# GRatTWCU/Social-STGCNN

Hardware: AMD Instinct MI355X
Metric: scene-windows/sec fwd+bwd (obs=8,pred=12) (higher is better)
Workload: dtype f32; 1 GPU; synthetic V=32 scene-windows, obs 8 / pred 12, batch 2048 per GPU, f32 (BASELINE north-star: V<=32, batch=2048; SURVEY 8d generator); global_batch=2048, step=aggregation + forward + bivariate NLL + backward + SGD update, parallelism=dp1

## Files before the change

### social_stgcnn_amd/csrc/model_bwd.hip

```cpp
#include "model_common.hpp"
#include "stgcn_block.hpp"
#include "txp_scene_common.hpp"
#include "step_plan.hpp"
#include "txp_wgrad.hpp"
#include "tail_parts.hpp"
#include "nll_elem.hpp"

namespace stg {

struct BwdArgs {
    ModelLayout lay;
    const float *params, *buffers, *x;
    int64_t x_sn, x_sc, x_st, x_sv;
    const float *adj;
    int64_t a_sn;
    const int32_t *num_peds;
    int N, V;
    const float *dy, *ws;
    const float *nll_target, *nll_weights;
    float *nll_losses;
    int64_t ws_stride;
    float *slab1;
    float *dzg;
    float *dx;
// ... 221 lines not shown
                const int r = e / vi, w = e - r * vi;
                dcur[e] = dyn[(int64_t)r * V + w];
            }
            __syncthreads();
        }
        float *H1 = dzb, *DH2 = dzb + C * (T + 2) * Vl, *DB1 = DH2 + C * (T + 2) * Vl;
        for (int j = L.n_blocks - 1; j >= 0 && !STG_SKIP(a, 4); --j) {
            const float *xin = j > 0 ? wsn + L.ws_hdr_floats + (int64_t)L.blk[j - 1].ws_s * V : nullptr;
            float *dxs = j > 0 ? dcur : nullptr;
            float *dxg = j == 0 ? dxn : nullptr;
            if (L.blk[j].cin == Cfg::CIN0)
                stgcn_block_bwd<Cfg::CIN0, WAVES, true>(a, params, L.blk[j], n, vi, dcur, H1, DH2, DB1, red, tot, gsm, wsn,
                                                        xin, dxs, dxg, nullptr);
            else
                stgcn_block_bwd<Cfg::C, WAVES, true>(a, params, L.blk[j], n, vi, dcur, H1, DH2, DB1, red, tot, gsm, wsn, xin,
                                                     dxs, dxg, nullptr);
        }
    }
    __syncthreads();
    float *slab = a.slab1 + (int64_t)blockIdx.x * n_small;
    for (int e = tid; e < n_small; e += NT) slab[e] = gsm[e];
}

struct ReduceSeg {
    int p0, len, rows, row_stride;
    int64_t base;
};
struct ReduceArgs {
    ReduceSeg seg[kMaxTxp + 3];
    int n_seg;
    const float *slabs;
    float *grad;
    int n_params;
};

struct TailArgs {
    float *params;
    const float *lr_dev;
    float lr;
    const float *stats, *losses, *weights;
    const int32_t *num_peds;
    float *buffers, *total;
    NbtPtrs nbt;
    int n_reduce, n_buffers, N, stat_floats;
    float momentum;
};

__global__ __launch_bounds__(256) void reduce_slabs_kernel(const ReduceArgs a, const TailArgs t_) {
    __shared__ float part[32][8];
    if ((int)blockIdx.x >= t_.n_reduce) {
        float *acc_s = &part[0][0];
        __shared__ float dec_s[256];
        __shared__ int cnt_s[256];
        const int b = (int)blockIdx.x - t_.n_reduce;
        if (b < t_.n_buffers)
            bn_fold_body<256>(b, t_.stats, t_.num_peds, t_.N, t_.stat_floats, t_.momentum, t_.buffers, t_.nbt, acc_s, dec_s,
                              cnt_s);
        else if (t_.total)
            weighted_sum_body(t_.losses, t_.weights, t_.N, t_.total, acc_s);
        return;
    }
    const int col = threadIdx.x & 7, grp = threadIdx.x >> 3;
    const int p = blockIdx.x * 8 + col;
    float s = 0.f;
    if (p < a.n_params) {
        for (int q = 0; q < a.n_seg; ++q) {
            const ReduceSeg g = a.seg[q];
            if (p >= g.p0 && p < g.p0 + g.len) {
                const float *src = a.slabs + g.base + (p - g.p0);
                int k = grp;
                for (; k + 992 < g.rows; k += 1024) {
                    float v[32];
#pragma unroll
                    for (int u = 0; u < 32; ++u) v[u] = src[(int64_t)(k + 32 * u) * g.row_stride];
#pragma unroll
                    for (int u = 0; u < 32; ++u) s += v[u];
                }
                for (; k + 480 < g.rows; k += 512) {
                    float v[16];
#pragma unroll
                    for (int u = 0; u < 16; ++u) v[u] = src[(int64_t)(k + 32 * u) * g.row_stride];
#pragma unroll
                    for (int u = 0; u < 16; ++u) s += v[u];
                }
                for (; k + 96 < g.rows; k += 128) {
                    float v[4];
#pragma unroll
                    for (int u = 0; u < 4; ++u) v[u] = src[(int64_t)(k + 32 * u) * g.row_stride];
#pragma unroll
                    for (int u = 0; u < 4; ++u) s += v[u];
                }
                for (; k < g.rows; k += 32) s += src[(int64_t)k * g.row_stride];
            }
        }
    }
    part[grp][col] = s;
    __syncthreads();
    if (grp == 0 && p < a.n_params) {
        float t = 0.f;
#pragma unroll
        for (int g = 0; g < 32; ++g) t += part[g][col];
        a.grad[p] = t;
        if (t_.params) t_.params[p] -= (t_.lr_dev ? t_.lr_dev[0] : t_.lr) * t;
    }
}

static int env_waves(const char *name, int dflt) {
    const int w = diag_env(name, dflt);
    return (w == 1 || w == 2 || w == 4 || w == 8) ? w : dflt;
}

static size_t bwd_lds_bytes(const ModelLayout &L, int V, int waves) {
    const int plane = Cfg::P * txp_sc(V);
    const int st = (2 * Cfg::C * (Cfg::T + 2) + Cfg::C * Cfg::T) * V;
    const int reg = plane > st ? plane : st;
    const int dcur = Cfg::P * Cfg::C * V;
    const int n_small = L.n_blk_params + L.n_txp;
    const size_t fl = ((n_small + 3) & ~3) + (size_t)reg + (size_t)dcur + (size_t)waves * kRedMax + kRedMax;
    return fl * sizeof(float);
}

static int bwd_waves(const StepPath &path, int V) {
    return path.wg_waves ? path.wg_waves : (V <= 40 ? 1 : (V <= 80 ? 4 : 8));
}

static int bwd_grid_w(const ModelLayout &L, int N, int V, int waves) {
    const size_t lds = bwd_lds_bytes(L, V, waves);
// ... 91 lines not shown
        return STG_EUNSUPPORTED;
    STG_REQUIRE(!(path.scene() && dx), STG_EUNSUPPORTED,
                "stg_model_bwd: dx is only computed by the workgroup-per-scene kernels: set STG_OPT_WG_PATH in the "
                "descriptor of the forward and the backward call");
    a.params = params; a.buffers = buffers; a.x = x;
    a.x_sn = x_sn; a.x_sc = x_sc; a.x_st = x_st; a.x_sv = x_sv;
    a.adj = adj; a.a_sn = a_sn; a.num_peds = num_peds; a.N = N; a.V = V;
    a.nll_target = nll_target; a.nll_weights = nll_weights; a.nll_losses = nll_losses;
    a.dy = dy; a.ws = ws; a.ws_stride = ws_floats_per_scene(L, V); a.slab1 = rows; a.dzg = dzg; a.dx = dx;
    int32_t *order = reinterpret_cast<int32_t *>(scratch + cv.order);
    bool sorted;
    const WsTail wt = ws_tail(L, path, N, V);
    const float *ws_end = ws + wt.base;
    if (tail_has_order(path, num_peds, N, V)) {
        order = reinterpret_cast<int32_t *>(const_cast<float *>(ws_end) + wt.order);
        sorted = true;
    } else {
        sorted = launch_scene_order(num_peds, N, V, order, order + N, st, order + N + V + 2);
    }
    int32_t *order_peds = order + N + V + 2;
    const int serp = diag_env("STG_WALK", 1);
    a.tier = SceneTier{sorted ? order : nullptr, sorted ? order + N : nullptr, -1, V, serp};
    a.debug_skip = diag_env("STG_DEBUG_SKIP", 0);
    int slab_rows;
    if (path.scene()) {
        TxpBwdArgs t{};
        t.lay = L; t.params = params; t.num_peds = num_peds; t.N = N; t.V = V; t.dy = dy; t.ws = ws;
        t.nll_target = nll_target; t.nll_weights = nll_weights; t.nll_losses = nll_losses;
        t.x = x; t.x_sn = x_sn; t.x_sc = x_sc; t.x_st = x_st; t.x_sv = x_sv; t.adj = adj; t.a_sn = a_sn;
        t.ws_stride = a.ws_stride; t.dzg = dzg; t.rows = rows;
        t.tier = a.tier;
        t.Vl = V;
        t.debug_skip = a.debug_skip;
        t.split_bf16 = (L.flags & STG_OPT_SPLIT_BF16) ? 1 : 0;
        t.stagger = diag_env("STG_STAGGER_B", 0);
        if (wt.wp >= 0) t.wp = reinterpret_cast<const unsigned *>(ws_end + wt.wp);
        const int rcw = launch_scene_bwd(path, t, st);
        if (rcw != STG_OK) return rcw;
        slab_rows = N;
    } else {
        const int waves = bwd_waves(path, V);
        const size_t lds = bwd_lds_bytes(L, V, waves);
        STG_REQUIRE(lds <= (size_t)kLdsBytes, STG_ELDS, "stg_model_bwd: V=%d needs %zu bytes of LDS (> %d)", V, lds,
                    kLdsBytes);
        const int grid = bwd_grid(L, path, N, V);
        void (*k1)(BwdArgs, const float *);
        switch (waves) {
            case 1: k1 = model_bwd_kernel<1>; break;
            case 2: k1 = model_bwd_kernel<2>; break;
            case 4: k1 = model_bwd_kernel<4>; break;
            default: k1 = model_bwd_kernel<8>; break;
        }
        slab_rows = grid;
        const int grid_small = a.tier.order ? bwd_grid_small(L, N, V) : 0;
        if (grid_small > 0) a.tier.v_lo = kBwdTierV;
        int rck = launch(Launch{"stg_model_bwd: K1", dim3(grid), dim3(waves * 64), lds, st}, k1, a, params);
        if (rck != STG_OK) return rck;
        if (grid_small > 0) {
            a.Vl = kBwdTierV;
            a.tier.v_lo = -1; a.tier.v_hi = kBwdTierV;
            a.slab1 = rows + (int64_t)grid * n_small;
            rck = launch(Launch{"stg_model_bwd: K1 (small scenes)", dim3(grid_small), dim3(64), bwd_lds_bytes(L, kBwdTierV, 1), st},
                         model_bwd_kernel<1>, a, params);
            if (rck != STG_OK) return rck;
            slab_rows = grid + grid_small;
            a.slab1 = rows;
            a.Vl = 0;
            a.tier.v_hi = V;
        }
    }
    evl.mark();

    ReduceArgs r{};
    r.slabs = scratch;
    r.grad = grad_params;
    r.n_params = L.n_params;
    r.seg[r.n_seg++] = ReduceSeg{0, L.n_blk_params, slab_rows, n_small, cv.rows};
    if (L.n_txp > 0) {
        r.seg[r.n_seg++] = ReduceSeg{L.prelus, L.n_txp, slab_rows, n_small, cv.rows + (int64_t)L.n_blk_params};
        WgradArgs w{};
        w.lay = L; w.num_peds = num_peds; w.order = a.tier.order; w.order_peds = sorted ? order_peds : nullptr;
        w.key_start = a.tier.key_start;
        w.serpentine = a.tier.serpentine; w.N = N; w.V = V;
        w.ws = ws; w.dzg = dzg; w.ws_stride = a.ws_stride; w.slab2 = slab2; w.rows = wg.rows; w.debug_skip = a.debug_skip;
        for (int l = 0; l <= L.L + 1; ++l) w.wg_begin[l] = wg.wg_begin[l];
        if (!STG_SKIP(a, 1)) {
            const int rck = launch_txp_wgrad(w, wg, st);
            if (rck != STG_OK) return rck;
        }
        evl.mark();
        for (int l = 0; l <= L.L; ++l) {
            const int p0 = l == L.L ? L.out_w : L.txp_w[l];
            r.seg[r.n_seg++] = ReduceSeg{p0, wgrad_row_len(l), STG_SKIP(a, 1) ? 0 : wg.wg_begin[l + 1] - wg.wg_begin[l],
                                         wgrad_row_len(l), cv.slab2 + wgrad_slab_base(l, wg.rows)};
        }
    }
    TailArgs ta{};
    ta.n_reduce = (L.n_params + 7) / 8;
    int extra = 0;
    if (tail) {
        ta.params = tail->params; ta.lr_dev = tail->lr_dev; ta.lr = tail->lr;
        ta.stats = tail->stats; ta.buffers = tail->buffers; ta.total = tail->total;
        ta.losses = nll_losses; ta.weights = nll_weights; ta.num_peds = num_peds;
        ta.N = N; ta.stat_floats = L.stat_floats; ta.momentum = d->bn_momentum;
        ta.n_buffers = (tail->stats && N > 0) ? L.n_buffers : 0;
        ta.nbt.n = tail->nbt ? tail->n_bn : 0;
        for (int k = 0; k < ta.nbt.n; ++k) ta.nbt.p[k] = tail->nbt[k];
        extra = ta.n_buffers + 1;
    }
    hipLaunchKernelGGL(reduce_slabs_kernel, dim3(ta.n_reduce + extra), dim3(256), 0, st, r, ta);
    STG_LAUNCH_CHECK("stg_model_bwd: reduce_slabs");
    evl.mark();
    evl.finish();
    return STG_OK;
}

int stg_model_bwd(const stg_model_desc *d, const float *params, const float *buffers, const float *x, int64_t x_sn,
                  int64_t x_sc, int64_t x_st, int64_t x_sv, const float *adj, int64_t a_sn, const int32_t *num_peds,
                  int N, int V, const float *dy, const float *ws, float *scratch, float *grad_params, float *dx,
                  void **events, int n_events, void *stream) {
    return model_bwd_impl(d, params, buffers, x, x_sn, x_sc, x_st, x_sv, adj, a_sn, num_peds, N, V, dy, nullptr, nullptr,
                          nullptr, nullptr, ws, scratch, grad_params, dx, events, n_events, stream);
}

int stg_model_bwd_nll(const stg_model_desc *d, const float *params, const float *buffers, const float *x, int64_t x_sn,
                      int64_t x_sc, int64_t x_st, int64_t x_sv, const float *adj, int64_t a_sn, const int32_t *num_peds,
                      int N, int V, const float *y, const float *target, const float *weights, float *losses,
                      const float *ws, float *scratch, float *grad_params, void **events, int n_events, void *stream) {
    if (!target || !losses || (N > 0 && !y)) return stg::fail(STG_EINVAL, "stg_model_bwd_nll: null pointer");
    return model_bwd_impl(d, params, buffers, x, x_sn, x_sc, x_st, x_sv, adj, a_sn, num_peds, N, V, y, target, weights,
                          losses, nullptr, ws, scratch, grad_params, nullptr, events, n_events, stream);
// ... 17 lines not shown
```

### social_stgcnn_amd/csrc/tail_parts.hpp

```cpp
#pragma once
#include "model_common.hpp"

namespace stg {

struct NbtPtrs {
    int64_t *p[3 * STG_MAX_BLOCKS];
    int n;
};

template <int NT>
__device__ __forceinline__ void bn_fold_body(int i, const float *__restrict__ stats, const int32_t *__restrict__ num_peds,
                                             int N, int stat_floats, float momentum, float *__restrict__ buffers,
                                             const NbtPtrs &nbt, float *acc_s, float *dec_s, int *cnt_s) {
    const int tid = threadIdx.x;
    const int chunk = (N + NT - 1) / NT;
    const int lo = tid * chunk, hi = (lo + chunk) < N ? (lo + chunk) : N;
    const float keep = 1.0f - momentum;
    float acc = 0.f, dec = 1.f;
    int cnt = 0;
    for (int n0 = lo; n0 < hi; n0 += 8) {
        float sv[8];
        bool live[8];
#pragma unroll
        for (int u = 0; u < 8; ++u) {
// ... 86 lines not shown
        acc = wave_sum(acc);
        if ((tid & 63) == 0) red[tid >> 6] = acc;
        __syncthreads();
        float tot = 0.f;
        for (int w = 0; w < (nt >> 6); ++w) tot += red[w];
        const float nrm = sqrtf(tot);
        if (norm_out && tid == 0) norm_out[0] = nrm;
        if (max_norm > 0.f) {
            coef = max_norm / (nrm + 1e-6f);
            coef = coef > 1.f ? 1.f : coef;
        }
    }
    for (int64_t i = tid; i < n; i += nt) {
        float gi = g[i];
        if (max_norm > 0.f) {
            gi *= coef;
            g[i] = gi;
        }
        p[i] = p[i] - lr * gi;
    }
}

__device__ __forceinline__ void weighted_sum_body(const float *__restrict__ v, const float *__restrict__ w, int N,
                                                  float *__restrict__ out, float *red ) {
    const int tid = threadIdx.x;
    float acc = 0.f;
    for (int i = tid; i < N; i += blockDim.x) acc = w ? fmaf(v[i], w[i], acc) : acc + v[i];
    acc = wave_sum(acc);
    if ((tid & 63) == 0) red[tid >> 6] = acc;
    __syncthreads();
    if (tid == 0) {
        float t = 0.f;
        for (int k = 0; k < (int)(blockDim.x >> 6); ++k) t += red[k];
        out[0] = t;
    }
}

}
```

### social_stgcnn_amd/csrc/txp_scene_common.hpp

```cpp
#pragma once
#include "model_common.hpp"
#include "stgcn_block.hpp"

namespace stg {

struct MixGeom {
    int on;
    int v_small, v_mid;
    int block_floats;
};

constexpr int kTeamMaxV = 128;
struct TeamGeom {
    int on;
    int v1, v2;
    int region_floats;
};

struct TxpFwdArgs {
    ModelLayout lay;
    const float *params, *buffers;
    const int32_t *num_peds;
    SceneTier tier;
    int Vl;
// ... 21 lines not shown
    const float *params;
    const int32_t *num_peds;
    SceneTier tier;
    int Vl;
    MixGeom mix;
    TeamGeom team;
    int N, V;
    const float *x;
    int64_t x_sn, x_sc, x_st, x_sv;
    const float *adj;
    int64_t a_sn;
    const float *dy;
    const float *nll_target;
    const float *nll_weights;
    float *nll_losses;
    const float *ws;
    int64_t ws_stride;
    float *dzg;
    const unsigned *wp;
    float *rows;
    int debug_skip;
    int split_bf16;
    int stagger;
};

bool txp_fwd_x6_fits(const ModelLayout &L, int V);
bool txp_bwd_x6_fits(const ModelLayout &L, int V);
int64_t txp_bwd_x6_wp_floats(const ModelLayout &L);
int launch_txp_fwd_x6(const TxpFwdArgs &a, hipStream_t st);
int launch_txp_bwd_x6(const TxpBwdArgs &a, hipStream_t st);

__host__ __device__ inline int ptab_floats(int v) { return ((Cfg::T * v + 1) / 2 + 3) & ~3; }
__host__ __device__ inline int bwd_ptab_floats(int v) { return ptab_floats(v) + kRedMax; }
__host__ __device__ inline int wave_param_floats(const ModelLayout &L) {
    return ((L.n_blk_params + 3) & ~3) + ((L.n_buffers + 3) & ~3);
}

__device__ __forceinline__ void build_ptab(ptab_t *ptab, int vi) {
    const int lane = threadIdx.x & 63;
    for (int p = lane; p < Cfg::T * vi; p += 64) {
        const int h = p / vi;
        ptab[p] = (ptab_t)((h << 8) | (p - h * vi));
    }
}
__device__ __forceinline__ void build_ptab(ptab_t *ptab, int w0, int wc) {
    const int lane = threadIdx.x & 63;
// ... 38 lines not shown
```

### social_stgcnn_amd/csrc/txp_wgrad.hip

```cpp
#include "txp_wgrad.hpp"

namespace stg {

namespace {

constexpr int C = Cfg::C, P = Cfg::P;
constexpr int kWaves = 8;

__device__ __forceinline__ void wait_vmcnt(int n) {
    switch (n) {
        case 0: asm volatile("s_waitcnt vmcnt(0)" ::: "memory"); break;
        case 1: asm volatile("s_waitcnt vmcnt(1)" ::: "memory"); break;
        case 2: asm volatile("s_waitcnt vmcnt(2)" ::: "memory"); break;
        case 3: asm volatile("s_waitcnt vmcnt(3)" ::: "memory"); break;
        case 4: asm volatile("s_waitcnt vmcnt(4)" ::: "memory"); break;
        case 5: asm volatile("s_waitcnt vmcnt(5)" ::: "memory"); break;
        case 6: asm volatile("s_waitcnt vmcnt(6)" ::: "memory"); break;
        case 7: asm volatile("s_waitcnt vmcnt(7)" ::: "memory"); break;
        case 8: asm volatile("s_waitcnt vmcnt(8)" ::: "memory"); break;
        default: asm volatile("s_waitcnt vmcnt(0)" ::: "memory"); break;
    }
}

__device__ __forceinline__ void dma_piece(const float *__restrict__ src, float *lds_dst, int nvec, int piece) {
// ... 243 lines not shown
        per_cu = (int)((size_t)kLdsBytes / g->lds);
    }
    int total = kNumCU * per_cu;
    if (const int v = diag_env("STG_WGRAD_GRID", 0)) total = v > 0 ? v : total;
    const int nl = L.L + 1;
    if (total < nl) total = nl;
    const int need = N * wgrad_chunks(V);
    const int w0 = g->bf16mma ? 15 : 6, w1 = g->bf16mma ? 18 : 7, wsum = w0 + w1 * (nl - 1);
    int begin = 0, maxw = 0;
    for (int l = 0; l < nl; ++l) {
        int cnt = (int)((int64_t)total * (l == 0 ? w0 : w1) / wsum);
        if (cnt < 1) cnt = 1;
        if (cnt > need) cnt = need;
        g->wg_begin[l] = begin;
        begin += cnt;
        if (cnt > maxw) maxw = cnt;
    }
    g->wg_begin[nl] = begin;
    g->grid = begin;
    g->rows = maxw;
    return true;
}

int launch_txp_wgrad(const WgradArgs &w, const WgradGeom &g, hipStream_t st) {
    if (g.bf16mma) return launch_txp_wgrad_bf16(w, g, st);
    const Launch lc{"txp_wgrad", dim3(g.grid), dim3(kWaves * 64), g.lds, st};
    const bool bf16 = (w.lay.flags & STG_OPT_BF16_STORE) != 0;
    if (g.nbuf == 3)
        return launch(lc, bf16 ? txp_wgrad_kernel<3, true> : txp_wgrad_kernel<3, false>, w, w.order, w.order_peds, w.num_peds);
    return launch(lc, bf16 ? txp_wgrad_kernel<4, true> : txp_wgrad_kernel<4, false>, w, w.order, w.order_peds, w.num_peds);
}

}
```

### social_stgcnn_amd/csrc/txp_wgrad.hpp

```cpp
#pragma once
#include "model_common.hpp"

namespace stg {

constexpr int kWgradChunkV = 32;
__host__ __device__ inline int wgrad_chunks(int V) { return (V + kWgradChunkV - 1) / kWgradChunkV; }
__host__ __device__ inline int wgrad_image_v(int V) { return V < kWgradChunkV ? V : kWgradChunkV; }
__host__ __device__ inline int wgrad_plane_floats(int V0, bool bf16) {
    const int V = wgrad_image_v(V0);
    if (!bf16) return plane_slot(V);
    return (((Cfg::C + 2) * save_sw(V, true) * Cfg::P) / 2 + 3) & ~3;
}
__host__ __device__ inline int wgrad_image_floats(int V0, bool bf16 = false) {
    const int V = wgrad_image_v(V0);
    if (!bf16) return plane_slot(V) + dz_slot(V);
    return wgrad_plane_floats(V0, true) + (((Cfg::C * save_vw(V, true) * Cfg::P) / 2 + 3 + 4) & ~3);
}
__host__ __device__ inline int wgrad_row_len(int layer) {
    return Cfg::P * (layer == 0 ? Cfg::T : Cfg::P) * 9 + Cfg::P;
}
__host__ __device__ inline int64_t wgrad_slab_base(int layer, int rows) {
    return layer == 0 ? 0 : (int64_t)rows * (wgrad_row_len(0) + (int64_t)(layer - 1) * wgrad_row_len(1));
}

// ... 1 lines not shown
    int waves, nbuf, grid, rows;
    bool bf16mma;
    int wg_begin[kMaxTxp + 2];
    size_t lds;
};
bool wgrad_geom(const ModelLayout &L, int N, int V, WgradGeom *g);

struct WgradArgs {
    ModelLayout lay;
    const int32_t *num_peds;
    const int32_t *order;
    const int32_t *order_peds;
    const int32_t *key_start;
    int serpentine;
    int N, V;
    const float *ws;
    const float *dzg;
    int64_t ws_stride;
    float *slab2;
    int rows;
    int wg_begin[kMaxTxp + 2];
    int debug_skip;
};
int launch_txp_wgrad(const WgradArgs &w, const WgradGeom &g, hipStream_t st);
bool wgrad_bf16_fits(const ModelLayout &L, int V);
void wgrad_bf16_geom(WgradGeom *g, const ModelLayout &L, int V);
int launch_txp_wgrad_bf16(const WgradArgs &w, const WgradGeom &g, hipStream_t st);

}
```

### social_stgcnn_amd/csrc/txp_wgrad_bf16.hip

```cpp
#include "txp_conv_bf16.hpp"
#include "txp_wgrad.hpp"
#include "scene_team.hpp"
#include <type_traits>

namespace stg {

namespace {

constexpr int C = Cfg::C, P = Cfg::P;
constexpr int kRec = 96;
constexpr int kPiece = 32;
constexpr int SWI = kWgradChunkV + 2, VWI = kWgradChunkV;
constexpr int kARecs = (C + 2) * SWI;
constexpr int kZRecs = C * VWI;
constexpr int kZeroRec = kARecs + kZRecs;
constexpr int kOnesRec = kZeroRec + 1;
constexpr int kImageBytes = (kOnesRec + 1) * kRec;
constexpr int kATasks = C * SWI * 3, kZTasks = C * VWI * 3;

typedef unsigned u32x2 __attribute__((ext_vector_type(2)));
typedef unsigned u32x4 __attribute__((ext_vector_type(4)));

struct Item {
    int vc, w0;
// ... 280 lines not shown
                    if (jj < 9 * CINL) row[(co * CINL + ci) * 9 + tap] = acc[k][r];
                    else if (jj == 9 * CINL) row[P * CINL * 9 + co] = acc[k][r];
                }
            }
        }
    }
    __syncthreads();
    const int len = wgrad_row_len(layer);
    float *dst = a.slab2 + wgrad_slab_base(layer, a.rows) + (int64_t)wg * len;
    for (int e = tid; e < len; e += NTH) {
        int jj = 9 * CINL;
        if (e < P * CINL * 9) {
            const int tap = e % 9, ci = (e / 9) % CINL;
            jj = tap * CINL + ci;
        }
        const int h = (jj >> 4) >= T0 ? 1 : 0;
        float t = 0.f;
#pragma unroll
        for (int sidx = 0; sidx < 5; ++sidx) t += rowsm[(sidx * HS + h) * ROW + e];
        dst[e] = t;
    }
}

template <bool BF, bool CH, int NW, int NIMG>
__global__ __launch_bounds__(NW * 64, NW == 5 ? 5 : 6) void txp_wgrad_bf16_kernel(const WgradArgs a, const int32_t *__restrict__ order,
                                                                   const int32_t *__restrict__ order_peds,
                                                                   const int32_t *__restrict__ num_peds,
                                                                   const int32_t *__restrict__ key_start) {
    extern __shared__ __attribute__((aligned(16))) unsigned char smb[];
    int l = 0;
    while (l < a.lay.L && (int)blockIdx.x >= a.wg_begin[l + 1]) ++l;
    const int wg = (int)blockIdx.x - a.wg_begin[l];
    const int nwg = a.wg_begin[l + 1] - a.wg_begin[l];
    if (l == 0)
        layer<Cfg::T, BF, CH, NW, NIMG>(a, order, order_peds, num_peds, key_start, l, smb, wg, nwg);
    else
        layer<Cfg::P, BF, CH, NW, NIMG>(a, order, order_peds, num_peds, key_start, l, smb, wg, nwg);
}


}

bool wgrad_bf16_fits(const ModelLayout &L, int V) {
    (void)V;
    return !(L.flags & STG_OPT_F32_MFMA);
}

void wgrad_bf16_geom(WgradGeom *g, const ModelLayout &L, int V) {
    (void)V;
    const bool bf = (L.flags & STG_OPT_BF16_STORE) != 0;
    g->waves = bf ? 5 : 10;
    g->nbuf = bf ? 1 : 2;
    const size_t row = (size_t)((Cfg::P * Cfg::P * 9 + Cfg::P + 3) & ~3) * sizeof(float) * g->waves;
    size_t lds = (size_t)g->nbuf * kImageBytes;
    if (lds < row) lds = row;
    g->lds = lds;
}

template <bool B, int NW, int NI>
static auto wgrad_bf16_kernel(bool ch) { return ch ? txp_wgrad_bf16_kernel<B, true, NW, NI> : txp_wgrad_bf16_kernel<B, false, NW, NI>; }

int launch_txp_wgrad_bf16(const WgradArgs &w, const WgradGeom &g, hipStream_t st) {
    const Launch lc{"txp_wgrad_bf16", dim3(g.grid), dim3(g.waves * 64), g.lds, st};
    const bool bf = (w.lay.flags & STG_OPT_BF16_STORE) != 0, ch = w.V > kWgradChunkV;
    const bool five = g.waves == 5 && g.nbuf == 1, ten = g.waves == 10 && g.nbuf == 2;
#ifdef STG_K2_ALL_SHAPES
    if (five || ten) {
        const auto k = five ? (bf ? wgrad_bf16_kernel<true, 5, 1>(ch) : wgrad_bf16_kernel<false, 5, 1>(ch))
                            : (bf ? wgrad_bf16_kernel<true, 10, 2>(ch) : wgrad_bf16_kernel<false, 10, 2>(ch));
        return launch(lc, k, w, w.order, w.order_peds, w.num_peds, w.key_start);
    }
#else
    if (bf ? five : ten)
        return launch(lc, bf ? wgrad_bf16_kernel<true, 5, 1>(ch) : wgrad_bf16_kernel<false, 10, 2>(ch), w, w.order, w.order_peds,
                      w.num_peds, w.key_start);
#endif
    return fail(STG_EINVAL, "txp_wgrad_bf16: no kernel for %d waves / %d images", g.waves, g.nbuf);
}

}
```

### social_stgcnn_amd/csrc/txp_x6.hip

```cpp
#include "txp_scene_common.hpp"
#include "nll_elem.hpp"
#include "txp_conv_bf16.hpp"

namespace stg {

namespace {

constexpr int C = Cfg::C, P = Cfg::P, T = Cfg::T;

enum class Shape { Generic, Canon, Canon32 };
constexpr int kCanonV = 32;
constexpr int64_t kCanonWs32 = ws_floats_per_scene(kCanonLayout, kCanonV);
constexpr int64_t kCanonAggStride32[2] = {(int64_t)(Cfg::CIN0 + 1) * Cfg::T * kCanonV, kCanonWs32};
constexpr int64_t kCanonAggAx32[2] = {0, kCanonLayout.ws_hdr_floats + (int64_t)kCanonLayout.blk[0].ws_ax * kCanonV};
constexpr int64_t kCanonAggCs32[2] = {(int64_t)Cfg::CIN0 * Cfg::T * kCanonV,
                                      kCanonLayout.ws_hdr_floats + (int64_t)kCanonLayout.blk[0].ws_cs * kCanonV};

template <Shape S, typename Args>
__device__ __forceinline__ void fold_shape(Args &a) {
    if constexpr (S != Shape::Generic) {
        ModelLayout k = kCanonLayout;
        k.eps = a.lay.eps;
        k.momentum = a.lay.momentum;
        k.bn_mode = a.lay.bn_mode;
// ... 200 lines not shown
    unsigned char *img = reinterpret_cast<unsigned char *>(region);
    const cv::LaneGeom lg = cv::lane_geom(vi, kX6Slots);
    constexpr bool bf16 = BF;
    const int VWs = save_vw(vi, bf16);
    auto tile_slots = [&](int t, int &rec, int &quad) {
        const int p = 16 * t + nq;
        const unsigned hw = ptab[p < npos ? p : 0];
        const int h = (int)(hw >> 8), w = (int)(hw & 0xffu);
        quad = (h * VWs + w) * 3 + kq;
        rec = (p < npos && kq < 3) ? cv::pos_off(vi, 1 + h, w) + 8 * kq : -1;
    };
    {
        uint4 *z4 = reinterpret_cast<uint4 *>(img);
        for (int e = lane + 64 * ck.ci(); e < cv::image_bytes(vi, kX6Slots) >> 4; e += 64 * ck.nch()) z4[e] = make_uint4(0u, 0u, 0u, 0u);
    }
    build_ptab(ptab, ck.w0(), ck.wc());
    ck.sync();
    f32x4 dcur[kX6Tiles];
#pragma unroll
    for (int t = 0; t < kX6Tiles; ++t) dcur[t] = f32x4{0.f, 0.f, 0.f, 0.f};

    for (int l = L.L; l >= 0; --l) {
        float *dzo = a.dzg + ((int64_t)n * (L.L + 1) + l) * dz_slot(V);
        if (STG_SKIP(a, 512) || (l == L.L && STG_SKIP(a, 2048)) || (l != L.L && STG_SKIP(a, 4096))) {
        } else if (l == L.L) {
            const int wcw = ck.wc();
            const int vp = wcw <= 1 ? 1 : (wcw <= 2 ? 2 : (wcw <= 4 ? 4 : (wcw <= 8 ? 8 : (wcw <= 16 ? 16 : 32))));
            const int sh = __builtin_ctz(vp), rpi = 64 >> sh;
            const int sub = lane >> sh, wl = lane & (vp - 1), w = ck.w0() + wl;
            const bool okw = wl < wcw;
            float *S = reinterpret_cast<float *>(img + lg.PL);
            auto put1 = [&](int rc, float g) { S[rc * vi + w] = g; };
            if (a.nll_target) {
                const float *tn = a.nll_target + (int64_t)n * P * V * 2;
                const float inv_cnt = 1.0f / (float)(P * vi);
                const float gs = inv_cnt * (a.nll_weights ? a.nll_weights[n] : 1.f);
                float lacc = 0.f;
#pragma unroll 1
                for (int p0 = 0; p0 < P; p0 += rpi) {
                    const int p = p0 + sub;
                    if (okw && p < P) {
                        const float *q = dyn + (int64_t)p * V + w;
                        const float2 tg = *reinterpret_cast<const float2 *>(tn + ((int64_t)p * V + w) * 2);
                        float g[5];
#ifdef STG_DIAG
                        if (STG_SKIP(a, 1 << 21))
// ... 36 lines not shown
#pragma unroll
            for (int t = 0; t < kX6Tiles; ++t) {
                const int p = 16 * t + nq;
                const unsigned hw = ptab[p < npos ? p : 0];
                const float *sq = S + ((4 * (kq < 3 ? kq : 0)) * C + (int)(hw >> 8)) * vi + (int)(hw & 0xffu);
                qd[t] = f32x4{sq[0], sq[C * vi], sq[2 * C * vi], sq[3 * C * vi]};
            }
            ck.sync();
            {
                uint4 *z4 = reinterpret_cast<uint4 *>(img + lg.PL);
                for (int e = lane + 64 * ck.ci(); e < (2 * lg.PL + 128) >> 4; e += 64 * ck.nch()) z4[e] = make_uint4(0u, 0u, 0u, 0u);
            }
            ck.sync();
            int rec[kX6Tiles], qv[kX6Tiles];
#pragma unroll
            for (int t = 0; t < kX6Tiles; ++t) tile_slots(t, rec[t], qv[t]);
#pragma unroll
            for (int t = 0; t < kX6Tiles; ++t) {
                if (rec[t] >= 0) {
                    cv::put4(img, (unsigned)rec[t], lg.PL, qd[t]);
                    store_vec4(dzo, qv[t], qd[t], bf16);
                }
            }
        } else {
            const float *zl = wsn + L.ws_hdr_floats + (int64_t)lay_ws_z<SH>(L, l) * V;
            const float alpha = Pm[L.prelus + l];
            float slope_acc = 0.f;
            f32x4 zv[kX6Tiles];
            int rec[kX6Tiles], qv[kX6Tiles];
#pragma unroll
            for (int t = 0; t < kX6Tiles; ++t) tile_slots(t, rec[t], qv[t]);
#pragma unroll
            for (int t = 0; t < kX6Tiles; ++t)
                zv[t] = rec[t] >= 0 ? load_vec4_raw(zl, qv[t], bf16) : f32x4{1.f, 1.f, 1.f, 1.f};
            asm volatile("" ::"v"(zv[0]), "v"(zv[1]), "v"(zv[2]), "v"(zv[3]), "v"(zv[4]), "v"(zv[5]), "v"(zv[6]), "v"(zv[7]),
                         "v"(zv[8]), "v"(zv[9]), "v"(alpha)
                         : "memory");
            vm_drain();
#pragma unroll
            for (int t = 0; t < kX6Tiles; ++t) {
                if (rec[t] >= 0) {
                    f32x4 dzv;
                    const f32x4 zq = finish_vec4(zv[t], bf16);
#pragma unroll
                    for (int r = 0; r < 4; ++r) {
                        const float z = zq[r], d = dcur[t][r];
                        float dz = d;
                        if (!(z > 0.f)) {
                            dz = alpha * d;
                            slope_acc = fmaf(d, z, slope_acc);
                        }
                        dzv[r] = dz;
                    }
                    cv::put4(img, (unsigned)rec[t], lg.PL, dzv);
                    store_vec4(dzo, qv[t], dzv, bf16);
                }
            }
            float ss[1] = {slope_acc};
            ck.template reduce<1>(ss);
            if (ck.writer()) prow[L.n_blk_params + l] = ss[0];
        }
        ck.sync();
        if (!STG_SKIP(a, 1024)) {
            cv::u32x4 w[cv::kWpVecs];
            cv::load_wp(a.wp + (int64_t)l * cv::kWpDwords, w);
            asm volatile("" ::"v"(w[0]), "v"(w[cv::kWpVecs - 1]) : "memory");
            vm_drain();
            const unsigned lds_base = (unsigned)(uintptr_t)img;
            const bool keep = l != L.L && l != 0;
            const f32x4 zero = {0.f, 0.f, 0.f, 0.f};
            unsigned code = cv::tile_code(0, ptab, npos);
#pragma unroll
            for (int t = 0; t < kX6Tiles; ++t) {
                if (t < ntiles) {
                    const cv::Tile tl = cv::tile_from<1>(t, code, npos, lg, vi);
                    if (t + 1 < kX6Tiles) code = cv::tile_code(t + 1, ptab, npos);
                    cv::BHalf b;
                    f32x4 acc = keep ? dcur[t] : zero;
                    cv::load_b_half<0>(lds_base, tl, b);
                    cv::mma_half<0>(w, b, acc);
                    cv::load_b_half<1>(lds_base, tl, b);
                    cv::mma_half<1>(w, b, acc);
                    dcur[t] = acc;
                }
            }
        }
        ck.sync();
    }
// ... 10 lines not shown
    }
    __builtin_amdgcn_wave_barrier();
    if constexpr (!CK::kTeam) {
        for (int e = L.L + lane; e < L.n_txp; e += 64) slope_row[e] = 0.f;
    }
    if (!STG_SKIP(a, 4))
        stgcn_block_bwd_cols<true>(a, blk_params, L.blk[0], n, vi, D, slope_row - L.n_blk_params, a.ws + n * a.ws_stride, ck);
    if constexpr (CK::kTeam) {
        ck.sync();
        if (ck.lead()) {
            float *row = slope_row - L.n_blk_params;
            const int nrow = L.n_blk_params + L.n_txp;
            for (int e0 = 0; e0 < kTeamRow; e0 += 64) {
                const int e = e0 + lane < kTeamRow ? e0 + lane : kTeamRow - 2;
                float t = ck.row_of(0)[e];
                for (int c = 1; c < ck.nch(); ++c) t += ck.row_of(c)[e];
                if (e < nrow) row[e] = t;
                if (e == kTeamRowLoss && a.nll_target) a.nll_losses[n] = t * (1.0f / (float)(P * vi));
            }
        }
    }
}

template <int WPB, bool BF, Shape S>
__global__ __launch_bounds__(WPB * 64, WPB == 8 ? 1 : 2) __attribute__((amdgpu_waves_per_eu(2, 2))) void txp_bwd_x6_kernel(
    const TxpBwdArgs a0) {
    extern __shared__ __attribute__((aligned(16))) float sm[];
    TxpBwdArgs a = a0;
    fold_shape<S>(a);
    const int Vl = a.Vl, wave = threadIdx.x >> 6;
    const int per_wave = bwd6_region_floats(Vl) + bwd_ptab_floats(Vl);
    float *region = sm + wave * per_wave;
    ptab_t *ptab = reinterpret_cast<ptab_t *>(region + bwd6_region_floats(Vl));
    float *blk_p = sm + WPB * per_wave;
    stage_block_params(a.lay, a.params, nullptr, blk_p, nullptr, WPB * 64);
    const int gw = __builtin_amdgcn_readfirstlane(blockIdx.x * WPB + wave), nw = gridDim.x * WPB;
    int begin, end;
    tier_range(a.tier, a.N, a.V, begin, end);
    const int M = end - begin;
    for (int r = 0; r * nw < M; ++r) {
        const int it = walk_item(r, gw, nw, M, a.tier.order != nullptr && a.tier.serpentine);
        if (it < 0) continue;
        const int n = __builtin_amdgcn_readfirstlane(a.tier.order ? scene_index(a.tier.order[begin + it], a.N) : it);
        int vi = a.num_peds ? a.num_peds[n] : a.V;
        vi = __builtin_amdgcn_readfirstlane(vi < 0 ? 0 : (vi > a.V ? a.V : vi));
        txp_bwd_scene_x6<BF, SoloScene, S>(a, blk_p, n, vi, region, ptab, SoloScene{vi});
        __builtin_amdgcn_wave_barrier();
    }
}

struct TeamCount {
    int n4, n2, n1;
// ... 65 lines not shown
    float *blk_p = xr + 2 * kXrFwd, *blk_b = blk_p + ((a.lay.n_blk_params + 3) & ~3);
    stage_block_params(a.lay, params, buffers, blk_p, blk_b, 256);
    const TeamCount tc = team_count(a.tier, a.team, a.num_peds, a.N, a.V);
    const int G = team_workers(tc.units, gridDim.x);
    int prev = 1;
    for (int r = 0; r * G < tc.units; ++r) {
        const int u = walk_item(r, blockIdx.x, G, tc.units, a.tier.serpentine != 0);
        if (u < 0 || (int)blockIdx.x >= G) continue;
        const TeamUnit q = team_unit(a.tier, tc, a.num_peds, a.N, a.V, u);
        if (q.nch > 1 || prev > 1) team_barrier();
        prev = q.nch;
        if (q.n >= 0) {
            const TeamScene ck{q.vi, q.w0, q.wc, q.nch, q.ci, xr + (q.slot & 1) * kXrFwd, nullptr, q.nch > 1 && !STG_SKIP(a, 1 << 20)};
            float *region = sm + q.slot * ((R >> 2) * q.nch);
            txp_fwd_scene_x6<BF>(a, params, blk_p, blk_b, q.n, q.vi, region, ptab, ck);
        }
        __builtin_amdgcn_wave_barrier();
    }
}

template <bool BF>
__global__ __launch_bounds__(256, 2) __attribute__((amdgpu_waves_per_eu(2, 2))) void txp_bwd_team_kernel(const TxpBwdArgs a) {
    extern __shared__ __attribute__((aligned(16))) float sm[];
    const int wave = __builtin_amdgcn_readfirstlane(threadIdx.x >> 6);
    const int R = a.team.region_floats;
    ptab_t *ptab = reinterpret_cast<ptab_t *>(sm + R + wave * team_ptab_floats());
    float *xr = sm + R + 4 * team_ptab_floats();
    float *blk_p = xr + kXrBwdWg;
    stage_block_params(a.lay, a.params, nullptr, blk_p, nullptr, 256);
    const TeamCount tc = team_count(a.tier, a.team, a.num_peds, a.N, a.V);
    const int G = team_workers(tc.units, gridDim.x);
    int prev = 1;
    for (int r = 0; r * G < tc.units; ++r) {
        const int u = walk_item(r, blockIdx.x, G, tc.units, a.tier.serpentine != 0);
        if (u < 0 || (int)blockIdx.x >= G) continue;
        const TeamUnit q = team_unit(a.tier, tc, a.num_peds, a.N, a.V, u);
        if (q.nch > 1 || prev > 1) team_barrier();
        prev = q.nch;
        if (q.n >= 0) {
            const TeamScene ck{q.vi, q.w0, q.wc, q.nch, q.ci, xr + (q.slot & 1) * kXrRows,
                               xr + 2 * kXrRows + q.slot * q.nch * kTeamRow, q.nch > 1 && !STG_SKIP(a, 1 << 20)};
            float *region = sm + q.slot * ((R >> 2) * q.nch);
            txp_bwd_scene_x6<BF>(a, blk_p, q.n, q.vi, region, ptab, ck);
        }
        __builtin_amdgcn_wave_barrier();
    }
// ... 122 lines not shown
```

Before: 9.438 million scene-windows/s.

## Fold slab reduction and SGD tail into the bf16 wgrad kernel via atomic counters

When the bf16 MFMA wgrad path is active, the cross-workgroup reduction of weight-gradient slabs, the small-parameter column reductions, BN buffer folding and loss sum are merged into the wgrad kernel. Last-arriving workgroups, detected with atomic counters, do the sums and apply the SGD update, and the counters are zeroed by the preceding bwd kernel. This removes the separate reduce_slabs kernel launch and its extra pass over the slabs, at the cost of serial tail work on a few workgroups and more fence/atomic synchronisation. It also moves the wp weight load earlier so it overlaps the dz store work.

```diff
diff --git a/social_stgcnn_amd/csrc/model_bwd.hip b/social_stgcnn_amd/csrc/model_bwd.hip
--- a/social_stgcnn_amd/csrc/model_bwd.hip
+++ b/social_stgcnn_amd/csrc/model_bwd.hip
@@ -267,30 +267,6 @@
     for (int e = tid; e < n_small; e += NT) slab[e] = gsm[e];
 }
 
-struct ReduceSeg {
-    int p0, len, rows, row_stride;
-    int64_t base;
-};
-struct ReduceArgs {
-    ReduceSeg seg[kMaxTxp + 3];
-    int n_seg;
-    const float *slabs;
-    float *grad;
-    int n_params;
-};
-
-struct TailArgs {
-    float *params;
-    const float *lr_dev;
-    float lr;
-    const float *stats, *losses, *weights;
-    const int32_t *num_peds;
-    float *buffers, *total;
-    NbtPtrs nbt;
-    int n_reduce, n_buffers, N, stat_floats;
-    float momentum;
-};
-
 __global__ __launch_bounds__(256) void reduce_slabs_kernel(const ReduceArgs a, const TailArgs t_) {
     __shared__ float part[32][8];
     if ((int)blockIdx.x >= t_.n_reduce) {
@@ -305,49 +281,7 @@
             weighted_sum_body(t_.losses, t_.weights, t_.N, t_.total, acc_s);
         return;
     }
-    const int col = threadIdx.x & 7, grp = threadIdx.x >> 3;
-    const int p = blockIdx.x * 8 + col;
-    float s = 0.f;
-    if (p < a.n_params) {
-        for (int q = 0; q < a.n_seg; ++q) {
-            const ReduceSeg g = a.seg[q];
-            if (p >= g.p0 && p < g.p0 + g.len) {
-                const float *src = a.slabs + g.base + (p - g.p0);
-                int k = grp;
-                for (; k + 992 < g.rows; k += 1024) {
-                    float v[32];
-#pragma unroll
-                    for (int u = 0; u < 32; ++u) v[u] = src[(int64_t)(k + 32 * u) * g.row_stride];
-#pragma unroll
-                    for (int u = 0; u < 32; ++u) s += v[u];
-                }
-                for (; k + 480 < g.rows; k += 512) {
-                    float v[16];
-#pragma unroll
-                    for (int u = 0; u < 16; ++u) v[u] = src[(int64_t)(k + 32 * u) * g.row_stride];
-#pragma unroll
-                    for (int u = 0; u < 16; ++u) s += v[u];
-                }
-                for (; k + 96 < g.rows; k += 128) {
-                    float v[4];
-#pragma unroll
-                    for (int u = 0; u < 4; ++u) v[u] = src[(int64_t)(k + 32 * u) * g.row_stride];
-#pragma unroll
-                    for (int u = 0; u < 4; ++u) s += v[u];
-                }
-                for (; k < g.rows; k += 32) s += src[(int64_t)k * g.row_stride];
-            }
-        }
-    }
-    part[grp][col] = s;
-    __syncthreads();
-    if (grp == 0 && p < a.n_params) {
-        float t = 0.f;
-#pragma unroll
-        for (int g = 0; g < 32; ++g) t += part[g][col];
-        a.grad[p] = t;
-        if (t_.params) t_.params[p] -= (t_.lr_dev ? t_.lr_dev[0] : t_.lr) * t;
-    }
+    reduce_cols_body<false>(a, t_, (int)blockIdx.x, part);
 }
 
 static int env_waves(const char *name, int dflt) {
@@ -485,6 +419,10 @@
     const int serp = diag_env("STG_WALK", 1);
     a.tier = SceneTier{sorted ? order : nullptr, sorted ? order + N : nullptr, -1, V, serp};
     a.debug_skip = diag_env("STG_DEBUG_SKIP", 0);
+    unsigned *fold_ctr = nullptr;
+    if (tail && path.scene() && path.bwd_x6 && L.n_txp > 0 && !STG_SKIP(a, 1) && wgrad_can_fold(wg, L) &&
+        order_floats(N, V) >= wgrad_fold_ctr_words(L) && !diag_env("STG_NO_FOLD", 0))
+        fold_ctr = reinterpret_cast<unsigned *>(scratch + cv.order);
     int slab_rows;
     if (path.scene()) {
         TxpBwdArgs t{};
@@ -498,6 +436,7 @@
         t.split_bf16 = (L.flags & STG_OPT_SPLIT_BF16) ? 1 : 0;
         t.stagger = diag_env("STG_STAGGER_B", 0);
         if (wt.wp >= 0) t.wp = reinterpret_cast<const unsigned *>(ws_end + wt.wp);
+        if (fold_ctr) { t.wipe = fold_ctr; t.n_wipe = wgrad_fold_ctr_words(L); }
         const int rcw = launch_scene_bwd(path, t, st);
         if (rcw != STG_OK) return rcw;
         slab_rows = N;
@@ -534,6 +473,19 @@
     }
     evl.mark();
 
+    TailArgs ta{};
+    ta.n_reduce = (L.n_params + 7) / 8;
+    int extra = 0;
+    if (tail) {
+        ta.params = tail->params; ta.lr_dev = tail->lr_dev; ta.lr = tail->lr;
+        ta.stats = tail->stats; ta.buffers = tail->buffers; ta.total = tail->total;
+        ta.losses = nll_losses; ta.weights = nll_weights; ta.num_peds = num_peds;
+        ta.N = N; ta.stat_floats = L.stat_floats; ta.momentum = d->bn_momentum;
+        ta.n_buffers = (tail->stats && N > 0) ? L.n_buffers : 0;
+        ta.nbt.n = tail->nbt ? tail->n_bn : 0;
+        for (int k = 0; k < ta.nbt.n; ++k) ta.nbt.p[k] = tail->nbt[k];
+        extra = ta.n_buffers + 1;
+    }
     ReduceArgs r{};
     r.slabs = scratch;
     r.grad = grad_params;
@@ -547,6 +499,29 @@
         w.serpentine = a.tier.serpentine; w.N = N; w.V = V;
         w.ws = ws; w.dzg = dzg; w.ws_stride = a.ws_stride; w.slab2 = slab2; w.rows = wg.rows; w.debug_skip = a.debug_skip;
         for (int l = 0; l <= L.L + 1; ++l) w.wg_begin[l] = wg.wg_begin[l];
+        if (fold_ctr) {
+            WgradFold f{};
+            f.ctr = fold_ctr;
+            for (int l = 0; l <= L.L; ++l) f.p0[l] = l == L.L ? L.out_w : L.txp_w[l];
+            f.small = r;
+            f.tail = ta;
+            int next = 0;
+            for (int q = 0; q < 2; ++q) {
+                const ReduceSeg &sg = r.seg[q];
+                int b0 = sg.p0 / 8, b1 = sg.len > 0 ? (sg.p0 + sg.len - 1) / 8 + 1 : b0;
+                if (b0 < next) b0 = next;
+                if (b1 < b0) b1 = b0;
+                f.blk0[q] = b0; f.nblk[q] = b1 - b0;
+                next = b1;
+            }
+            f.n_extra = f.nblk[0] + f.nblk[1] + extra;
+            const int rck = launch_txp_wgrad(w, wg, st, &f);
+            if (rck != STG_OK) return rck;
+            evl.mark();
+            evl.mark();
+            evl.finish();
+            return STG_OK;
+        }
         if (!STG_SKIP(a, 1)) {
             const int rck = launch_txp_wgrad(w, wg, st);
             if (rck != STG_OK) return rck;
@@ -557,19 +532,6 @@
             r.seg[r.n_seg++] = ReduceSeg{p0, wgrad_row_len(l), STG_SKIP(a, 1) ? 0 : wg.wg_begin[l + 1] - wg.wg_begin[l],
                                          wgrad_row_len(l), cv.slab2 + wgrad_slab_base(l, wg.rows)};
         }
-    }
-    TailArgs ta{};
-    ta.n_reduce = (L.n_params + 7) / 8;
-    int extra = 0;
-    if (tail) {
-        ta.params = tail->params; ta.lr_dev = tail->lr_dev; ta.lr = tail->lr;
-        ta.stats = tail->stats; ta.buffers = tail->buffers; ta.total = tail->total;
-        ta.losses = nll_losses; ta.weights = nll_weights; ta.num_peds = num_peds;
-        ta.N = N; ta.stat_floats = L.stat_floats; ta.momentum = d->bn_momentum;
-        ta.n_buffers = (tail->stats && N > 0) ? L.n_buffers : 0;
-        ta.nbt.n = tail->nbt ? tail->n_bn : 0;
-        for (int k = 0; k < ta.nbt.n; ++k) ta.nbt.p[k] = tail->nbt[k];
-        extra = ta.n_buffers + 1;
     }
     hipLaunchKernelGGL(reduce_slabs_kernel, dim3(ta.n_reduce + extra), dim3(256), 0, st, r, ta);
     STG_LAUNCH_CHECK("stg_model_bwd: reduce_slabs");
diff --git a/social_stgcnn_amd/csrc/tail_parts.hpp b/social_stgcnn_amd/csrc/tail_parts.hpp
--- a/social_stgcnn_amd/csrc/tail_parts.hpp
+++ b/social_stgcnn_amd/csrc/tail_parts.hpp
@@ -132,18 +132,95 @@
 }
 
 __device__ __forceinline__ void weighted_sum_body(const float *__restrict__ v, const float *__restrict__ w, int N,
-                                                  float *__restrict__ out, float *red ) {
+                                                  float *__restrict__ out, float *red , int nt = 0) {
     const int tid = threadIdx.x;
+    if (nt == 0) nt = (int)blockDim.x;
     float acc = 0.f;
-    for (int i = tid; i < N; i += blockDim.x) acc = w ? fmaf(v[i], w[i], acc) : acc + v[i];
+    for (int i = tid; i < N; i += nt) acc = w ? fmaf(v[i], w[i], acc) : acc + v[i];
     acc = wave_sum(acc);
     if ((tid & 63) == 0) red[tid >> 6] = acc;
     __syncthreads();
     if (tid == 0) {
         float t = 0.f;
-        for (int k = 0; k < (int)(blockDim.x >> 6); ++k) t += red[k];
+        for (int k = 0; k < (nt >> 6); ++k) t += red[k];
         out[0] = t;
     }
 }
 
-}
+struct ReduceSeg {
+    int p0, len, rows, row_stride;
+    int64_t base;
+};
+struct ReduceArgs {
+    ReduceSeg seg[kMaxTxp + 3];
+    int n_seg;
+    const float *slabs;
+    float *grad;
+    int n_params;
+};
+struct TailArgs {
+    float *params;
+    const float *lr_dev;
+    float lr;
+    const float *stats, *losses, *weights;
+    const int32_t *num_peds;
+    float *buffers, *total;
+    NbtPtrs nbt;
+    int n_reduce, n_buffers, N, stat_floats;
+    float momentum;
+};
+
+__device__ __forceinline__ void store_grad(float *grad, const TailArgs &t_, const float *lr_dev, int p, float t) {
+    grad[p] = t;
+    if (t_.params) t_.params[p] -= (lr_dev ? lr_dev[0] : t_.lr) * t;
+}
+
+template <bool COVERED_ONLY>
+__device__ __forceinline__ void reduce_cols_body(const ReduceArgs &a, const TailArgs &t_, int blk, float (*part)[8]) {
+    const int col = threadIdx.x & 7, grp = threadIdx.x >> 3;
+    const int p = blk * 8 + col;
+    float s = 0.f;
+    bool covered = false;
+    if (p < a.n_params) {
+        for (int q = 0; q < a.n_seg; ++q) {
+            const ReduceSeg g = a.seg[q];
+            if (p >= g.p0 && p < g.p0 + g.len) {
+                covered = true;
+                const float *src = a.slabs + g.base + (p - g.p0);
+                int k = grp;
+                for (; k + 992 < g.rows; k += 1024) {
+                    float v[32];
+#pragma unroll
+                    for (int u = 0; u < 32; ++u) v[u] = src[(int64_t)(k + 32 * u) * g.row_stride];
+#pragma unroll
+                    for (int u = 0; u < 32; ++u) s += v[u];
+                }
+                for (; k + 480 < g.rows; k += 512) {
+                    float v[16];
+#pragma unroll
+                    for (int u = 0; u < 16; ++u) v[u] = src[(int64_t)(k + 32 * u) * g.row_stride];
+#pragma unroll
+                    for (int u = 0; u < 16; ++u) s += v[u];
+                }
+                for (; k + 96 < g.rows; k += 128) {
+                    float v[4];
+#pragma unroll
+                    for (int u = 0; u < 4; ++u) v[u] = src[(int64_t)(k + 32 * u) * g.row_stride];
+#pragma unroll
+                    for (int u = 0; u < 4; ++u) s += v[u];
+                }
+                for (; k < g.rows; k += 32) s += src[(int64_t)k * g.row_stride];
+            }
+        }
+    }
+    part[grp][col] = s;
+    __syncthreads();
+    if (grp == 0 && p < a.n_params && (covered || !COVERED_ONLY)) {
+        float t = 0.f;
+#pragma unroll
+        for (int g = 0; g < 32; ++g) t += part[g][col];
+        store_grad(a.grad, t_, t_.lr_dev, p, t);
+    }
+}
+
+}
diff --git a/social_stgcnn_amd/csrc/txp_scene_common.hpp b/social_stgcnn_amd/csrc/txp_scene_common.hpp
--- a/social_stgcnn_amd/csrc/txp_scene_common.hpp
+++ b/social_stgcnn_amd/csrc/txp_scene_common.hpp
@@ -67,6 +67,8 @@
     int debug_skip;
     int split_bf16;
     int stagger;
+    unsigned *wipe;
+    int n_wipe;
 };
 
 bool txp_fwd_x6_fits(const ModelLayout &L, int V);
diff --git a/social_stgcnn_amd/csrc/txp_wgrad.hip b/social_stgcnn_amd/csrc/txp_wgrad.hip
--- a/social_stgcnn_amd/csrc/txp_wgrad.hip
+++ b/social_stgcnn_amd/csrc/txp_wgrad.hip
@@ -289,8 +289,9 @@
     return true;
 }
 
-int launch_txp_wgrad(const WgradArgs &w, const WgradGeom &g, hipStream_t st) {
-    if (g.bf16mma) return launch_txp_wgrad_bf16(w, g, st);
+int launch_txp_wgrad(const WgradArgs &w, const WgradGeom &g, hipStream_t st, const WgradFold *fold) {
+    if (g.bf16mma) return launch_txp_wgrad_bf16(w, g, st, fold);
+    STG_REQUIRE(!fold, STG_EINVAL, "txp_wgrad: the fp32-MFMA kernel does not carry the reduction");
     const Launch lc{"txp_wgrad", dim3(g.grid), dim3(kWaves * 64), g.lds, st};
     const bool bf16 = (w.lay.flags & STG_OPT_BF16_STORE) != 0;
     if (g.nbuf == 3)
diff --git a/social_stgcnn_amd/csrc/txp_wgrad.hpp b/social_stgcnn_amd/csrc/txp_wgrad.hpp
--- a/social_stgcnn_amd/csrc/txp_wgrad.hpp
+++ b/social_stgcnn_amd/csrc/txp_wgrad.hpp
@@ -1,5 +1,6 @@
 #pragma once
 #include "model_common.hpp"
+#include "tail_parts.hpp"
 
 namespace stg {
 
@@ -47,9 +48,27 @@
     int wg_begin[kMaxTxp + 2];
     int debug_skip;
 };
-int launch_txp_wgrad(const WgradArgs &w, const WgradGeom &g, hipStream_t st);
+constexpr int kFoldCtrWords = 9;
+constexpr int kFoldMaxMembers = 255;
+struct WgradFold {
+    unsigned *ctr;
+    int32_t p0[kMaxTxp + 1];
+    ReduceArgs small;
+    TailArgs tail;
+    int blk0[2], nblk[2];
+    int n_extra;
+};
+__host__ __device__ inline int wgrad_fold_ctr_words(const ModelLayout &L) { return (L.L + 1) * kFoldCtrWords; }
+
+int launch_txp_wgrad(const WgradArgs &w, const WgradGeom &g, hipStream_t st, const WgradFold *fold = nullptr);
 bool wgrad_bf16_fits(const ModelLayout &L, int V);
 void wgrad_bf16_geom(WgradGeom *g, const ModelLayout &L, int V);
-int launch_txp_wgrad_bf16(const WgradArgs &w, const WgradGeom &g, hipStream_t st);
+int launch_txp_wgrad_bf16(const WgradArgs &w, const WgradGeom &g, hipStream_t st, const WgradFold *fold = nullptr);
+inline bool wgrad_can_fold(const WgradGeom &g, const ModelLayout &L) {
+    if (!g.bf16mma) return false;
+    for (int l = 0; l <= L.L; ++l)
+        if ((g.wg_begin[l + 1] - g.wg_begin[l] + 31) / 32 > kFoldMaxMembers) return false;
+    return true;
+}
 
 }
diff --git a/social_stgcnn_amd/csrc/txp_wgrad_bf16.hip b/social_stgcnn_amd/csrc/txp_wgrad_bf16.hip
--- a/social_stgcnn_amd/csrc/txp_wgrad_bf16.hip
+++ b/social_stgcnn_amd/csrc/txp_wgrad_bf16.hip
@@ -326,6 +326,91 @@
     }
 }
 
+template <int NTH>
+__device__ __forceinline__ void fold_layer(const WgradArgs &a, const WgradFold &f, int layer, int wg, int nwg, int *flag) {
+    const int tid = threadIdx.x;
+    const int len = wgrad_row_len(layer);
+    float *base = a.slab2 + wgrad_slab_base(layer, a.rows);
+    const int g = wg & 31, ng = nwg < 32 ? nwg : 32, members = (nwg - g + 31) >> 5;
+    unsigned *ctr = f.ctr + layer * kFoldCtrWords;
+    __threadfence();
+    __syncthreads();
+    if (tid == 0) {
+        const unsigned old = atomicAdd(ctr + (g >> 2), 1u << (8 * (g & 3)));
+        *flag = (int)((old >> (8 * (g & 3))) & 0xffu) == members - 1;
+    }
+    __syncthreads();
+    if (!*flag) return;
+    __threadfence();
+    for (int q = tid; q < (len >> 2); q += NTH) {
+        f32x4 s = {0.f, 0.f, 0.f, 0.f};
+#pragma unroll 4
+        for (int k = g; k < nwg; k += 32) s += *reinterpret_cast<const f32x4 *>(base + (int64_t)k * len + 4 * q);
+        *reinterpret_cast<f32x4 *>(base + (int64_t)g * len + 4 * q) = s;
+    }
+    __threadfence();
+    __syncthreads();
+    if (tid == 0) *flag = atomicAdd(ctr + kFoldCtrWords - 1, 1u) == (unsigned)(ng - 1);
+    __syncthreads();
+    if (!*flag) return;
+    __threadfence();
+    const float *lr_dev = f.tail.lr_dev;
+    for (unsigned p = tid; p < (unsigned)len; p += NTH) {
+        float t = 0.f;
+        for (int u0 = 0; u0 < ng; u0 += 16) {
+            float v[16];
+#pragma unroll
+            for (int u = 0; u < 16; ++u) v[u] = base[(unsigned)(u0 + u < ng ? u0 + u : u0) * (unsigned)len + p];
+#pragma unroll
+            for (int u = 0; u < 16; ++u) t += u0 + u < ng ? v[u] : 0.f;
+        }
+        store_grad(f.small.grad, f.tail, lr_dev, f.p0[layer] + p, t);
+    }
+}
+
+#ifndef STG_FOLD_EXTRAS_BEHIND
+constexpr bool kFoldExtrasInFront = true;
+#else
+constexpr bool kFoldExtrasInFront = false;
+#endif
+__device__ __forceinline__ void fold_extra(const WgradFold &f, int e, unsigned char *sm) {
+    if (threadIdx.x >= 256) return;
+    float(*part)[8] = reinterpret_cast<float(*)[8]>(sm);
+    float *acc_s = reinterpret_cast<float *>(sm), *dec_s = acc_s + 256;
+    int *cnt_s = reinterpret_cast<int *>(dec_s + 256);
+    if (e < f.nblk[0]) return reduce_cols_body<true>(f.small, f.tail, f.blk0[0] + e, part);
+    e -= f.nblk[0];
+    if (e < f.nblk[1]) return reduce_cols_body<true>(f.small, f.tail, f.blk0[1] + e, part);
+    e -= f.nblk[1];
+    const TailArgs &t_ = f.tail;
+    if (e < t_.n_buffers)
+        bn_fold_body<256>(e, t_.stats, t_.num_peds, t_.N, t_.stat_floats, t_.momentum, t_.buffers, t_.nbt, acc_s, dec_s, cnt_s);
+    else if (t_.total)
+        weighted_sum_body(t_.losses, t_.weights, t_.N, t_.total, acc_s, 256);
+}
+
+template <bool BF, bool CH, int NW, int NIMG>
+__global__ __launch_bounds__(NW * 64, NW == 5 ? 5 : 6) void txp_wgrad_bf16_fold_kernel(const WgradArgs a, const int32_t *__restrict__ order,
+                                                                        const int32_t *__restrict__ order_peds,
+                                                                        const int32_t *__restrict__ num_peds,
+                                                                        const int32_t *__restrict__ key_start,
+                                                                        const WgradFold f) {
+    extern __shared__ __attribute__((aligned(16))) unsigned char smb[];
+    const int n_main = (int)gridDim.x - f.n_extra;
+    const int ex = kFoldExtrasInFront ? (int)blockIdx.x : (int)blockIdx.x - n_main;
+    if (ex >= 0 && ex < f.n_extra) return fold_extra(f, ex, smb);
+    const int bx = kFoldExtrasInFront ? (int)blockIdx.x - f.n_extra : (int)blockIdx.x;
+    int l = 0;
+    while (l < a.lay.L && bx >= a.wg_begin[l + 1]) ++l;
+    const int wg = bx - a.wg_begin[l];
+    const int nwg = a.wg_begin[l + 1] - a.wg_begin[l];
+    if (l == 0)
+        layer<Cfg::T, BF, CH, NW, NIMG>(a, order, order_peds, num_peds, key_start, l, smb, wg, nwg);
+    else
+        layer<Cfg::P, BF, CH, NW, NIMG>(a, order, order_peds, num_peds, key_start, l, smb, wg, nwg);
+    fold_layer<NW * 64>(a, f, l, wg, nwg, reinterpret_cast<int *>(smb));
+}
+
 template <bool BF, bool CH, int NW, int NIMG>
 __global__ __launch_bounds__(NW * 64, NW == 5 ? 5 : 6) void txp_wgrad_bf16_kernel(const WgradArgs a, const int32_t *__restrict__ order,
                                                                    const int32_t *__restrict__ order_peds,
@@ -364,10 +449,20 @@
 template <bool B, int NW, int NI>
 static auto wgrad_bf16_kernel(bool ch) { return ch ? txp_wgrad_bf16_kernel<B, true, NW, NI> : txp_wgrad_bf16_kernel<B, false, NW, NI>; }
 
-int launch_txp_wgrad_bf16(const WgradArgs &w, const WgradGeom &g, hipStream_t st) {
-    const Launch lc{"txp_wgrad_bf16", dim3(g.grid), dim3(g.waves * 64), g.lds, st};
+template <bool B, int NW, int NI>
+static auto wgrad_bf16_fold_kernel(bool ch) { return ch ? txp_wgrad_bf16_fold_kernel<B, true, NW, NI> : txp_wgrad_bf16_fold_kernel<B, false, NW, NI>; }
+
+int launch_txp_wgrad_bf16(const WgradArgs &w, const WgradGeom &g, hipStream_t st, const WgradFold *fold) {
     const bool bf = (w.lay.flags & STG_OPT_BF16_STORE) != 0, ch = w.V > kWgradChunkV;
     const bool five = g.waves == 5 && g.nbuf == 1, ten = g.waves == 10 && g.nbuf == 2;
+    if (fold) {
+        STG_REQUIRE((bf ? five : ten) && fold->ctr && g.lds >= 4096, STG_EINVAL, "txp_wgrad_bf16: no folding kernel for %d waves / %d images",
+                    g.waves, g.nbuf);
+        const Launch lf{"txp_wgrad_bf16 (+ reduction)", dim3(g.grid + fold->n_extra), dim3(g.waves * 64), g.lds, st};
+        return launch(lf, bf ? wgrad_bf16_fold_kernel<true, 5, 1>(ch) : wgrad_bf16_fold_kernel<false, 10, 2>(ch), w, w.order,
+                      w.order_peds, w.num_peds, w.key_start, *fold);
+    }
+    const Launch lc{"txp_wgrad_bf16", dim3(g.grid), dim3(g.waves * 64), g.lds, st};
 #ifdef STG_K2_ALL_SHAPES
     if (five || ten) {
         const auto k = five ? (bf ? wgrad_bf16_kernel<true, 5, 1>(ch) : wgrad_bf16_kernel<false, 5, 1>(ch))
diff --git a/social_stgcnn_amd/csrc/txp_x6.hip b/social_stgcnn_amd/csrc/txp_x6.hip
--- a/social_stgcnn_amd/csrc/txp_x6.hip
+++ b/social_stgcnn_amd/csrc/txp_x6.hip
@@ -246,6 +246,15 @@
 
     for (int l = L.L; l >= 0; --l) {
         float *dzo = a.dzg + ((int64_t)n * (L.L + 1) + l) * dz_slot(V);
+        cv::u32x4 w[cv::kWpVecs];
+        bool w_asked = false;
+        auto ask_w = [&]() {
+            if (!w_asked && !STG_SKIP(a, 1024)) {
+                cv::load_wp(a.wp + (int64_t)l * cv::kWpDwords, w);
+                asm volatile("" ::: "memory");
+            }
+            w_asked = true;
+        };
         if (STG_SKIP(a, 512) || (l == L.L && STG_SKIP(a, 2048)) || (l != L.L && STG_SKIP(a, 4096))) {
         } else if (l == L.L) {
             const int wcw = ck.wc();
@@ -328,6 +337,7 @@
                     store_vec4(dzo, qv[t], qd[t], bf16);
                 }
             }
+            ask_w();
         } else {
             const float *zl = wsn + L.ws_hdr_floats + (int64_t)lay_ws_z<SH>(L, l) * V;
             const float alpha = Pm[L.prelus + l];
@@ -362,14 +372,14 @@
                     store_vec4(dzo, qv[t], dzv, bf16);
                 }
             }
+            ask_w();
             float ss[1] = {slope_acc};
             ck.template reduce<1>(ss);
             if (ck.writer()) prow[L.n_blk_params + l] = ss[0];
         }
         ck.sync();
         if (!STG_SKIP(a, 1024)) {
-            cv::u32x4 w[cv::kWpVecs];
-            cv::load_wp(a.wp + (int64_t)l * cv::kWpDwords, w);
+            ask_w();
             asm volatile("" ::"v"(w[0]), "v"(w[cv::kWpVecs - 1]) : "memory");
             vm_drain();
             const unsigned lds_base = (unsigned)(uintptr_t)img;
@@ -426,12 +436,18 @@
     }
 }
 
+__device__ __forceinline__ void wipe_words(const TxpBwdArgs &a) {
+    if (a.wipe && blockIdx.x == 0)
+        for (int e = threadIdx.x; e < a.n_wipe; e += blockDim.x) a.wipe[e] = 0u;
+}
+
 template <int WPB, bool BF, Shape S>
 __global__ __launch_bounds__(WPB * 64, WPB == 8 ? 1 : 2) __attribute__((amdgpu_waves_per_eu(2, 2))) void txp_bwd_x6_kernel(
     const TxpBwdArgs a0) {
     extern __shared__ __attribute__((aligned(16))) float sm[];
     TxpBwdArgs a = a0;
     fold_shape<S>(a);
+    wipe_words(a);
     const int Vl = a.Vl, wave = threadIdx.x >> 6;
     const int per_wave = bwd6_region_floats(Vl) + bwd_ptab_floats(Vl);
     float *region = sm + wave * per_wave;
@@ -543,6 +559,7 @@
 template <bool BF>
 __global__ __launch_bounds__(256, 2) __attribute__((amdgpu_waves_per_eu(2, 2))) void txp_bwd_team_kernel(const TxpBwdArgs a) {
     extern __shared__ __attribute__((aligned(16))) float sm[];
+    wipe_words(a);
     const int wave = __builtin_amdgcn_readfirstlane(threadIdx.x >> 6);
     const int R = a.team.region_floats;
     ptab_t *ptab = reinterpret_cast<ptab_t *>(sm + R + wave * team_ptab_floats());
```

Result: slower. 5.103 million scene-windows/s (-45.9%).
